# GeekAlexis/FastMOT

Hardware: AMD Instinct MI355X
Metric: end-to-end tracker FPS @1080p/50 dets (higher is better)
Workload: dtype f16

## Files before the change

fastmot_amd/_lib.py:

```python
import ctypes as C
import os
import sys
import weakref
from pathlib import Path

import numpy as np
from types import SimpleNamespace

from .utils.nv12 import NV12Frame
from .utils.jpeg import JPEGFrame, QT_ENTRIES, max_coefficients
from .utils.source import SourceFrame
from .utils.yuv import PlanarFrame, frame_bytes
from .utils.packed import PackedFrame, row_bytes
from .utils.bayer import BayerFrame
from .utils.deep import DeepFrame, deep_frame_bytes
from .utils.devarray import DeviceArrayFrame

LIB_PATH = Path(os.environ.get('FASTMOT_LIB_PATH', Path(__file__).parent / 'libfastmot_hip.so'))

c_int_p = C.POINTER(C.c_int)
_lib = None


class FastMOTHipError(RuntimeError):
# ... 396 lines not shown
        n_trk = len(arrs[1]) + len(arrs[3])
        out = np.empty(CASCADE_HEADER + 3 * n_trk + 3 * len(arrs[6]), np.int32)
        return cin, arrs, out

    def assoc_cascade(self, pack):
        cin, _, out = pack
        check(self.lib.fm_assoc_cascade(self._ctx, C.byref(cin), _ptr(out), C.c_int(len(out))))
        return out[:out[9]].tolist()

    def assoc_get_pairwise(self, nT, nD):
        feat = np.empty((nT, nD), np.float64)
        maha = np.empty((nT, nD), np.float64)
        iou = np.empty((nT, nD), np.float64)
        check(self.lib.fm_assoc_get_pairwise(self._ctx, _ptr(feat), _ptr(maha), _ptr(iou)))
        return feat, maha, iou

    def assoc_stage(self, stage, solver, rows, cols, motion_weight=0., max_cost=0., fill_val=1.,
                    row_labels=None, want_cost=False):
        r = _as(rows, np.int32)
        c = _as(cols, np.int32)
        nr, nc = len(r), len(c)
        mn = min(nr, nc)
        m_rows = np.empty(mn, np.int32)
        m_cols = np.empty(mn, np.int32)
        gated = np.zeros(mn, np.uint8)
        n_match = C.c_int(0)
        cost = np.empty((nr, nc), np.float64) if want_cost else None
        rl = _as(row_labels, np.int64) if row_labels is not None else None
        check(self.lib.fm_assoc_stage(self._ctx, C.c_int(stage), C.c_int(solver), C.c_int(nr), _ptr(r),
                                      C.c_int(nc), _ptr(c), C.c_double(motion_weight),
# ... 798 lines not shown
```

fastmot_amd/csrc/assoc.hip:

```cpp
#include "common.h"
#include "numba_set.h"
#include <algorithm>
#include <cmath>

namespace {

constexpr double INF_COST = 1e5;
constexpr double CHI_SQ_INV_95 = 9.4877;

__device__ inline double box_area(const double* b) {
    const double w = b[2] - b[0] + 1, h = b[3] - b[1] + 1;
    return (w <= 0 || h <= 0) ? 0. : w * h;
}

__device__ inline double iou_dist_pair(const double* a, double area_a, const double* b) {
    const double iw = fmin(a[2], b[2]) - fmax(a[0], b[0]) + 1;
    const double ih = fmin(a[3], b[3]) - fmax(a[1], b[1]) + 1;
    if (iw > 0 && ih > 0) {
        const double inter = iw * ih;
        const double uni = area_a + box_area(b) - inter;
        return 1. - inter / uni;
    }
    return 1.;
}
// ... 23 lines not shown
        }
        __syncthreads();
    }
    if (live) out[i] = occ;
}

__global__ void iou_dist_kernel(int na, const double* __restrict__ a, int nb,
                                const double* __restrict__ b, double* __restrict__ out) {
    const int idx = blockIdx.x * blockDim.x + threadIdx.x;
    if (idx >= na * nb) return;
    const int i = idx / nb, j = idx % nb;
    const double* pa = a + (size_t)i * 4;
    out[idx] = iou_dist_pair(pa, box_area(pa), b + (size_t)j * 4);
}

__global__ __launch_bounds__(256) void pairwise_kernel(
    int nT, int nD, int metric, int dim, const int32_t* __restrict__ slots,
    const double* __restrict__ trk_tlbr, const double* __restrict__ det_tlbr,
    const double* __restrict__ mean, const double* __restrict__ cov,
    const float* __restrict__ favg, const int32_t* __restrict__ fcnt,
    const float* __restrict__ emb, KFConst kf, const uint8_t* __restrict__ row_f32,
    double* __restrict__ feat, double* __restrict__ maha, double* __restrict__ iou,
    uint8_t* __restrict__ row_has_feat, char* __restrict__ mirror) {
    const size_t mat = (size_t)nT * nD;
    double* const mfeat = reinterpret_cast<double*>(mirror);
    extern __shared__ __attribute__((aligned(16))) char smem[];
    float* sa = reinterpret_cast<float*>(smem);
    double* sd = reinterpret_cast<double*>(smem + (size_t)dim * 4);
    const int t = blockIdx.x, tid = threadIdx.x;
    const int slot = slots[t];
    const int cnt = fcnt[slot];
    for (int k = tid; k < dim; k += 256) sa[k] = favg[(size_t)slot * dim + k];
    if (tid == 0) {
        const double* m = mean + (size_t)slot * 8;
        const double* P = cov + (size_t)slot * 64;
        const double w = m[2] - m[0] + 1, h = m[3] - m[1] + 1;
        const double sw = fmax(kf.fac_det[0] * w, kf.min_det[0]);
        const double sh = fmax(kf.fac_det[1] * h, kf.min_det[1]);
        double S[4][4], L[4][4];
        for (int i = 0; i < 4; ++i)
            for (int j = 0; j < 4; ++j) {
                S[i][j] = P[i * 8 + j];
                L[i][j] = 0.;
            }
        S[0][0] += sw * sw; S[1][1] += sh * sh; S[2][2] += sw * sw; S[3][3] += sh * sh;
        for (int j = 0; j < 4; ++j) {
            double s = S[j][j];
            for (int k = 0; k < j; ++k) s -= L[j][k] * L[j][k];
            L[j][j] = sqrt(s);
            for (int i = j + 1; i < 4; ++i) {
                double v = S[i][j];
                for (int k = 0; k < j; ++k) v -= L[i][k] * L[j][k];
                L[i][j] = v / L[j][j];
            }
        }
        for (int i = 0; i < 4; ++i) {
            for (int j = 0; j < 4; ++j) sd[i * 4 + j] = L[i][j];
            sd[16 + i] = m[i];
            sd[20 + i] = trk_tlbr[(size_t)t * 4 + i];
        }
        sd[24] = box_area(trk_tlbr + (size_t)t * 4);
        row_has_feat[t] = cnt > 0 ? 1 : 0;
        if (mirror) reinterpret_cast<uint8_t*>(mfeat + 3 * mat)[t] = cnt > 0 ? 1 : 0;
    }
    __syncthreads();
    for (int d = tid; d < nD; d += 256) {
        const double* z = det_tlbr + (size_t)d * 4;
        double y[4];
        for (int i = 0; i < 4; ++i) {
            double s = z[i] - sd[16 + i];
            for (int k = 0; k < i; ++k) s -= sd[i * 4 + k] * y[k];
            y[i] = s / sd[i * 4 + i];
        }
        const double md = y[0] * y[0] + y[1] * y[1] + y[2] * y[2] + y[3] * y[3];
        const double io = iou_dist_pair(sd + 20, sd[24], z);
        maha[(size_t)t * nD + d] = md;
        iou[(size_t)t * nD + d] = io;
        if (mirror) {
            mfeat[mat + (size_t)t * nD + d] = md;
            mfeat[2 * mat + (size_t)t * nD + d] = io;
        }
    }
    const int wv = tid >> 6, lane = tid & 63;
    const bool f32row = row_f32[t] != 0;
    if (cnt > 0) {
        for (int d = wv; d < nD; d += 4) {
            const float* b = emb + (size_t)d * dim;
            double acc0 = 0., acc1 = 0., acc2 = 0.;
            for (int k4 = lane; k4 < dim / 4; k4 += 64) {
                const float4 bv = *reinterpret_cast<const float4*>(b + k4 * 4);
                const float4 av = *reinterpret_cast<const float4*>(sa + k4 * 4);
                const float af[4] = {av.x, av.y, av.z, av.w};
                const float bf[4] = {bv.x, bv.y, bv.z, bv.w};
#pragma unroll
                for (int e = 0; e < 4; ++e) {
                    if (metric == FM_METRIC_COSINE) {
                        acc2 += (double)(bf[e] * bf[e]);
                        if (f32row) {
                            acc0 += (double)(af[e] * bf[e]);
                            acc1 += (double)(af[e] * af[e]);
                        } else {
                            const double a = af[e];
                            acc0 += a * (double)bf[e];
                            acc1 += a * a;
                        }
                    } else if (f32row) {
                        const float df = af[e] - bf[e];
                        acc0 += (double)(df * df);
                    } else {
                        const double dd = (double)af[e] - (double)bf[e];
                        acc0 += dd * dd;
                    }
                }
            }
            for (int off = 32; off > 0; off >>= 1) {
                acc0 += __shfl_xor(acc0, off);
                acc1 += __shfl_xor(acc1, off);
                acc2 += __shfl_xor(acc2, off);
            }
            if (lane == 0) {
                double v;
                if (metric == FM_METRIC_COSINE) v = 1. - acc0 / (sqrt(acc1) * sqrt(acc2));
                else v = sqrt(acc0);
                feat[(size_t)t * nD + d] = v;
                if (mirror) mfeat[(size_t)t * nD + d] = v;
            }
        }
    } else {
        for (int d = tid; d < nD; d += 256) {
            feat[(size_t)t * nD + d] = 1.;
            if (mirror) mfeat[(size_t)t * nD + d] = 1.;
        }
    }
}

__host__ __device__ inline double stage_cost(int stage, int t, int d, int nD, const double* __restrict__ feat,
                                             const double* __restrict__ maha, const double* __restrict__ iou,
                                             const uint8_t* __restrict__ row_has_feat, const uint8_t* __restrict__ docc,
                                             int64_t rlab, int64_t dlab, double motion_weight, double max_cost,
                                             double fill_val) {
    const size_t p = (size_t)t * nD + d;
    const bool lab_bad = rlab != dlab;
    double c;
    if (stage == FM_STAGE_MATCHING) {
        const bool empty = (!row_has_feat[t]) || docc[d];
        const double f = empty ? fill_val : feat[p];
// ... 500 lines not shown
    std::vector<size_t> offs;
    char* in = nullptr;
    int rc = upload(ctx, ctx->as_in,
                    {{slots, sizeof(int32_t) * nT}, {trk_tlbr, sizeof(double) * 4 * nT},
                     {trk_label, sizeof(int64_t) * nT}, {det_tlbr, sizeof(double) * 4 * nD},
                     {det_label, sizeof(int64_t) * nD}, {det_occluded, (size_t)nD},
                     {trk_feat_f32, (size_t)nT}}, offs, &in, early);
    if (rc) return rc;
    for (int i = 0; i < 6; ++i) ctx->as_off[i] = offs[i];
    const size_t mat = sizeof(double) * (size_t)nT * nD;
    if ((rc = ctx->as_pair.reserve(3 * mat + nT + 64))) return rc;
    char* pr = ctx->as_pair.dev<char>();
    const size_t shmem = (size_t)ctx->feat_dim * 4 + 32 * sizeof(double);
    if (after_extractor && !early) FM_HIP(hipStreamWaitEvent(ctx->s_main, ctx->ev_ext_net, 0));
    fm_trace_mark(ctx, st, 54);
    hipLaunchKernelGGL(pairwise_kernel, dim3(nT), dim3(256), shmem, st, nT, nD, metric,
                       ctx->feat_dim, (const int32_t*)(in + offs[0]), (const double*)(in + offs[1]),
                       (const double*)(in + offs[3]), ctx->mean, ctx->cov, ctx->feat_avg, ctx->feat_cnt,
                       ctx->emb, ctx->kf, (const uint8_t*)(in + offs[6]), (double*)pr, (double*)(pr + mat),
                       (double*)(pr + 2 * mat),
                       (uint8_t*)(pr + 3 * mat), mirror ? ctx->as_pair.host<char>() : nullptr);
    FM_HIP(hipGetLastError());
    fm_trace_mark(ctx, st, 55);
    if (mirror) FM_HIP(hipEventRecord(ctx->ev_pair, st));
    ctx->as_mirror = mirror;
    ctx->as_in_device = !early;
    ctx->as_in_bytes = offs[6] + (size_t)nT;
    return 0;
}

extern "C" int fm_assoc_prepare(fm_ctx* ctx, int metric, int nT, const int32_t* slots,
                                const double* trk_tlbr, const int64_t* trk_label, int nD,
                                const double* det_tlbr, const int64_t* det_label,
                                const uint8_t* det_occluded, const uint8_t* trk_feat_f32) {
    return assoc_prepare_impl(ctx, metric, nT, slots, trk_tlbr, trk_label, nD, det_tlbr, det_label, det_occluded,
                              trk_feat_f32, false);
// ... 250 lines not shown
}

extern "C" int fm_assoc_get_pairwise(fm_ctx* ctx, double* feat, double* maha, double* iou) {
    FM_CHECK_ARG(ctx);
    const size_t mat = sizeof(double) * (size_t)ctx->as_nT * ctx->as_nD;
    if (mat == 0) return 0;
    FM_HIP(hipStreamSynchronize(ctx->s_main));
    if (!ctx->as_in_device) FM_HIP(hipStreamSynchronize(ctx->s_ext));
    char* pr = ctx->as_pair.dev<char>();
    if (feat) FM_HIP(hipMemcpy(feat, pr, mat, hipMemcpyDeviceToHost));
    if (maha) FM_HIP(hipMemcpy(maha, pr + mat, mat, hipMemcpyDeviceToHost));
    if (iou) FM_HIP(hipMemcpy(iou, pr + 2 * mat, mat, hipMemcpyDeviceToHost));
    return 0;
}

extern "C" int fm_assoc_stage(fm_ctx* ctx, int stage, int solver, int nr, const int32_t* rows, int nc,
                              const int32_t* cols, double motion_weight, double max_cost,
                              double fill_val, const int64_t* row_label_override, int32_t* m_rows,
                              int32_t* m_cols, uint8_t* match_gated, int* n_match, double* cost_out) {
    FM_CHECK_ARG(ctx && n_match && nr >= 0 && nc >= 0);
    FM_CHECK_ARG(stage >= FM_STAGE_MATCHING && stage <= FM_STAGE_REID && (solver == 0 || solver == 1));
    *n_match = 0;
    if (nr == 0 || nc == 0) return 0;
    FM_CHECK_ARG(rows && cols && m_rows && m_cols);
    for (int i = 0; i < nr; ++i) FM_CHECK_ARG(rows[i] >= 0 && rows[i] < ctx->as_nT);
    for (int j = 0; j < nc; ++j) FM_CHECK_ARG(cols[j] >= 0 && cols[j] < ctx->as_nD);
    std::vector<int64_t> rlab(nr);
    if (row_label_override) memcpy(rlab.data(), row_label_override, sizeof(int64_t) * nr);
    else {
        const int64_t* tl = reinterpret_cast<const int64_t*>(ctx->as_in.host<char>() + ctx->as_off[2]);
// ... 37 lines not shown
```

fastmot_amd/csrc/common.h:

```cpp
#pragma once
#include <hip/hip_runtime.h>
#include <atomic>
#include <cstdarg>
#include <cstdint>
#include <cstdio>
#include <cstring>
#include <string>
#include <vector>
#include "../../include/fastmot_hip.h"
#ifdef FM_DIAG
#include "../../include/fastmot_hip_diag.h"
#endif

#define FM_ERR_HIP (-1)
#define FM_ERR_ARG (-2)
#define FM_ERR_STATE (-3)

void fm_set_error(const char* fmt, ...);

#define FM_HIP(call)                                                                        \
    do {                                                                                    \
        hipError_t e_ = (call);                                                             \
        if (e_ != hipSuccess) {                                                             \
            fm_set_error("%s:%d %s -> %s", __FILE__, __LINE__, #call, hipGetErrorString(e_)); \
// ... 61 lines not shown
struct SsdState;
struct GalleryState;
constexpr int FM_GALLERY_CHANNELS = 2;

struct fm_ctx {
    int device = 0;
    int opt_zero_copy_tracks = 2048;
    int opt_host_lap_elems = 262144;
    int opt_use_graphs = 1;
    int opt_fused_input = 1;
    int opt_net_timing = 0;
    int opt_nms_general = 0;
    int opt_det_front_ahead = 1;
    int opt_det_front_layers = -1;
    int opt_det_front_stream = 0;
    bool det_flush_deferred = false;
    int opt_lk_variant = 0;
    void* predict_worker = nullptr;
    hipStream_t s_main = nullptr;
    hipStream_t s_det = nullptr;
    hipStream_t s_up = nullptr;
    hipStream_t s_ext = nullptr;
    hipStream_t s_ext_x[FM_MAX_EXTRA_EXTRACTORS] = {};
    hipEvent_t ev_ext_in = nullptr, ev_ext_x_done[FM_MAX_EXTRA_EXTRACTORS] = {};
    hipStream_t s_flow = nullptr;
    hipStream_t s_flow2 = nullptr;
    hipEvent_t ev_pyr = nullptr;
    bool pyr_pending = false;
    hipEvent_t ev_prep = nullptr, ev_bg = nullptr;
    hipEvent_t ev_feat = nullptr;
// ... 186 lines not shown
```

fastmot_amd/csrc/ctx.hip:

```cpp
#include <algorithm>
#include "common.h"
void convd_set_cfg(int code);
#include <sched.h>
#include <cstring>
#include <cstdlib>
#include <cmath>

static thread_local char g_err[1024] = "";

void fm_set_error(const char* fmt, ...) {
    va_list ap;
    va_start(ap, fmt);
    vsnprintf(g_err, sizeof(g_err), fmt, ap);
    va_end(ap);
}

extern "C" const char* fm_last_error(void) { return g_err; }

extern "C" int fm_ctx_set_option(fm_ctx* ctx, const char* key, int value) {
    FM_CHECK_ARG(ctx && key && (value >= 0 || (value == -1 && !strcmp(key, "det_front_layers"))));
    if (!strcmp(key, "zero_copy_tracks")) ctx->opt_zero_copy_tracks = value;
    else if (!strcmp(key, "host_lap_elems")) ctx->opt_host_lap_elems = value;
    else if (!strcmp(key, "use_graphs")) ctx->opt_use_graphs = value;
    else if (!strcmp(key, "convd_cfg")) convd_set_cfg(value);
    else if (!strcmp(key, "nms_path")) {
        ctx->opt_nms_general = value != 0;
    }
    else if (!strcmp(key, "fused_input")) ctx->opt_fused_input = value != 0;
    else if (!strcmp(key, "net_timing")) ctx->opt_net_timing = value;
    else if (!strcmp(key, "det_front_ahead") || !strcmp(key, "det_front_stream")) {
        FM_CHECK_ARG(value <= (key[10] == 'a' ? 2 : 1));
        (key[10] == 'a' ? ctx->opt_det_front_ahead : ctx->opt_det_front_stream) = value;
    }
    else if (!strcmp(key, "det_front_layers")) ctx->opt_det_front_layers = value;
    else if (!strcmp(key, "lk_variant")) {
#ifndef FM_DIAG
        if (value != 0) {
            fm_set_error("option 'lk_variant' needs a diagnostic build of the library (-DFM_DIAG)");
            return FM_ERR_ARG;
        }
#endif
        ctx->opt_lk_variant = value;
    }
    else {
        fm_set_error("unknown option '%s'", key);
        return FM_ERR_ARG;
    }
    return 0;
}

extern "C" int fm_ctx_get_option(fm_ctx* ctx, const char* key, int* value) {
    FM_CHECK_ARG(ctx && key && value);
    if (!strcmp(key, "det_front_ahead")) *value = ctx->opt_det_front_ahead;
    else if (!strcmp(key, "det_front_layers")) *value = ctx->opt_det_front_layers;
    else if (!strcmp(key, "det_front_stream")) *value = ctx->opt_det_front_stream;
    else {
        fm_set_error("option '%s' cannot be read", key);
        return FM_ERR_ARG;
    }
    return 0;
}

extern "C" int fm_trace_start(fm_ctx* ctx, int cap, int64_t* host_ns) {
    FM_CHECK_ARG(ctx && cap > 0 && host_ns && !ctx->trace_on.load() && ctx->trace_ev.empty());
    FM_HIP(hipDeviceSynchronize());
    std::vector<hipEvent_t> evs(cap);
    for (auto& e : evs) FM_HIP(hipEventCreate(&e));
    if (!ctx->trace_base) FM_HIP(hipEventCreate(&ctx->trace_base));
    FM_HIP(hipEventRecord(ctx->trace_base, ctx->s_main));
    FM_HIP(hipEventSynchronize(ctx->trace_base));
// ... 54 lines not shown
    int n = 0;
    FM_HIP(hipGetDeviceCount(&n));
    if (device < 0 || device >= n) {
        fm_set_error("device %d out of range (%d visible)", device, n);
        return FM_ERR_ARG;
    }
    FM_HIP(hipSetDevice(device));
    fm_ctx* ctx = new fm_ctx();
    ctx->device = device;
    if (const char* e = getenv("FASTMOT_ZERO_COPY")) ctx->opt_zero_copy_tracks = atoi(e);
    if (const char* e = getenv("FASTMOT_HOST_LAP")) ctx->opt_host_lap_elems = atoi(e);
    if (const char* e = getenv("FASTMOT_GRAPHS")) ctx->opt_use_graphs = atoi(e);
    if (const char* e = getenv("FASTMOT_FUSED_INPUT")) ctx->opt_fused_input = atoi(e) != 0;
    if (const char* e = getenv("FASTMOT_FRONT_AHEAD")) ctx->opt_det_front_ahead = std::min(std::max(atoi(e), 0), 2);
    if (const char* e = getenv("FASTMOT_FRONT_STREAM")) ctx->opt_det_front_stream = atoi(e) == 1;
    int prio_lo = 0, prio_hi = 0;
    FM_HIP(hipDeviceGetStreamPriorityRange(&prio_lo, &prio_hi));
    const int prio_det = prio_lo, prio_ext = prio_hi;
    FM_HIP(hipStreamCreateWithPriority(&ctx->s_main, hipStreamNonBlocking, prio_hi));
    FM_HIP(hipStreamCreateWithPriority(&ctx->s_det, hipStreamNonBlocking, prio_det));
    FM_HIP(hipStreamCreateWithPriority(&ctx->s_up, hipStreamNonBlocking, prio_lo));
    FM_HIP(hipStreamCreateWithPriority(&ctx->s_ext, hipStreamNonBlocking, prio_ext));
    FM_HIP(hipEventCreateWithFlags(&ctx->ev_ext_in, hipEventDisableTiming));
    for (int i = 0; i < FM_MAX_EXTRA_EXTRACTORS; ++i) {
        FM_HIP(hipStreamCreateWithPriority(&ctx->s_ext_x[i], hipStreamNonBlocking, prio_hi));
        FM_HIP(hipEventCreateWithFlags(&ctx->ev_ext_x_done[i], hipEventDisableTiming));
    }
    FM_HIP(hipStreamCreateWithPriority(&ctx->s_flow, hipStreamNonBlocking, prio_hi));
    FM_HIP(hipStreamCreateWithPriority(&ctx->s_flow2, hipStreamNonBlocking, prio_hi));
    FM_HIP(hipEventCreateWithFlags(&ctx->ev_pyr, hipEventDisableTiming));
// ... 411 lines not shown
```

fastmot_amd/csrc/detect.hip:

```cpp
#include "pixel_source.h"
#include <cmath>
#include <string>
#include <vector>

struct DetState {
    fm_yolo_cfg cfg{};
    bool configured = false;
    int cap = 8192;
    static constexpr int NSLOT_UNTILED = FM_MAX_DET_BATCH + 2;
    static constexpr int NSLOT = 3 * FM_MAX_DET_BATCH;
    int nslot = NSLOT_UNTILED;
    int n_tiles = 0;
    int tile_x[FM_MAX_DET_BATCH] = {}, tile_y[FM_MAX_DET_BATCH] = {};
    int region_w = 0, region_h = 0;
    double tile_offset[FM_MAX_DET_BATCH][2] = {};
    double merge_thresh = 0.6;
    std::vector<fm_det48> tile_stage;
    std::vector<fm_det48> tile_dets;
    std::vector<int32_t> tile_ids;
    int tile_count[FM_MAX_DET_BATCH] = {};
    int tile_sum[2] = {};
    float* cand[NSLOT] = {};
    float* sorted[NSLOT] = {};
    int32_t* counters[NSLOT] = {};
    uint64_t* mask[NSLOT] = {};
    fm_det48* dets[NSLOT] = {};
    bool used[NSLOT] = {};
    hipEvent_t ev_dec[NSLOT] = {};
    int post_pending = -1;
    int post_pending_n = 0;
    bool general_post = false;
    static constexpr int GREEDY_RETRY = 1024;
    int general_passes = 0;
    int greedy_kmax = 2048, greedy_shrink = 0;
    bool sorted_valid[NSLOT] = {};
    static constexpr int PREFIX = 2048;
    fm_det48* dets_host[NSLOT] = {};
    int32_t* counters_host[NSLOT] = {};
    hipEvent_t ev_done[NSLOT] = {};
    hipStream_t s_fallback = nullptr;
    hipEvent_t ev0[NSLOT] = {}, ev1[NSLOT] = {};
    bool timed[NSLOT] = {};
    hipEvent_t evf0[NSLOT] = {}, evf1[NSLOT] = {};
    bool timed_front[NSLOT] = {};
    hipEvent_t ev_front[2] = {};
// ... 151 lines not shown
    const int i = blockIdx.x * blockDim.x + threadIdx.x;
    if (i >= n) return;
    const float* r = rows + (size_t)i * 7;
    emit_candidate(fa, r[0], r[1], r[2], r[3], r[4], (int)r[5], r[6], i);
}

#include "nms_core.h"

}
bool fm_det_defers_flush(fm_ctx* ctx) {
    return ctx->det && ctx->det_net && ctx->det_net->front_k > 0 && ctx->opt_det_front_ahead && ctx->opt_det_front_layers &&
           ctx->opt_det_front_stream == 0;
}
namespace {

int ensure_det(fm_ctx* ctx) {
    if (ctx->det) return 0;
    ctx->det = new DetState();
    return 0;
}

int alloc_post(DetState* d, int cap, int nslot) {
    cap = (cap + 63) & ~63;
    if (d->cand[0] && cap == d->cap && nslot == d->nslot) return 0;
    for (int i = (cap != d->cap || !d->cand[0]) ? 0 : nslot; i < DetState::NSLOT; ++i) {
        for (void* p : {(void*)d->cand[i], (void*)d->sorted[i], (void*)d->mask[i], (void*)d->dets[i]})
            if (p) (void)hipFree(p);
        if (d->dets_host[i]) (void)hipHostFree(d->dets_host[i]);
        d->dets_host[i] = nullptr;
        d->cand[i] = d->sorted[i] = nullptr; d->mask[i] = nullptr; d->dets[i] = nullptr;
    }
    for (int i = 0; i < DetState::NSLOT; ++i) d->used[i] = false;
    d->cap = cap;
    d->nslot = nslot;
    d->wr = d->rd = d->pending = 0;
    d->last = -1;
    d->post_pending = -1;
    d->post_pending_n = 0;
    d->set_slot[0] = d->set_slot[1] = -1;
    for (int i = 0; i < nslot; ++i) {
        if (d->cand[i]) continue;
        FM_HIP(hipMalloc(&d->cand[i], sizeof(float) * 8 * cap));
        FM_HIP(hipMalloc(&d->sorted[i], sizeof(float) * 8 * cap));
        FM_HIP(hipMalloc(&d->mask[i], sizeof(uint64_t) * (size_t)cap * (cap / 64)));
        FM_HIP(hipMalloc(&d->dets[i], sizeof(fm_det48) * cap));
        FM_HIP(hipHostMalloc(&d->dets_host[i], sizeof(fm_det48) * cap, hipHostMallocDefault));
    }
    for (int i = 0; i < nslot; ++i) {
        if (d->counters[i]) continue;
        FM_HIP(hipMalloc(&d->counters[i], sizeof(int32_t) * 4));
        FM_HIP(hipHostMalloc(&d->counters_host[i], sizeof(int32_t) * 4, hipHostMallocDefault));
        FM_HIP(hipEventCreateWithFlags(&d->ev_done[i], hipEventDisableTiming));
        FM_HIP(hipEventCreateWithFlags(&d->ev_dec[i], hipEventDisableTiming));
// ... 67 lines not shown
}

static int enqueue_greedy_post(fm_ctx* ctx, DetState* d, int slot, hipStream_t sp) {
    static bool configured = false;
    if (int rc = allow_dynamic_lds(nms_greedy_kernel, ng_lds_bytes(NG_KMAX), configured)) return rc;
    int rc = launch_rank_sort(d, slot, sp);
    if (rc) return rc;
    fm_trace_mark(ctx, sp, 22);
    const int kmax = d->greedy_kmax < d->cap ? d->greedy_kmax : (d->cap < NG_KMAX ? d->cap : NG_KMAX);
    hipLaunchKernelGGL(nms_greedy_kernel, dim3(1), dim3(NG_T), ng_lds_bytes(kmax), sp, d->sorted[slot], d->counters[slot],
                       d->cap, kmax, d->cfg.nms_thresh, post_out(d, slot));
    FM_HIP(hipGetLastError());
    return 0;
}

static int flush_post(fm_ctx* ctx, DetState* d) {
    const int first = d->post_pending, n = d->post_pending_n;
    if (first < 0) return 0;
    d->post_pending = -1;
    d->post_pending_n = 0;
    hipStream_t sp = ctx->s_up;
    FM_HIP(hipStreamWaitEvent(sp, d->ev_dec[first], 0));
    for (int i = 0; i < n; ++i) {
        const int slot = (first + i) % d->nslot;
        fm_trace_mark(ctx, sp, 20);
        int rc_p = (d->general_post || ctx->opt_nms_general) ? enqueue_general_post(ctx, d, slot, sp) : enqueue_greedy_post(ctx, d, slot, sp);
        if (rc_p) return rc_p;
        FM_HIP(hipEventRecord(d->ev_done[slot], sp));
        fm_trace_mark(ctx, sp, 21);
    }
    return 0;
}

int enqueue_post(fm_ctx* ctx, DetState* d, hipStream_t s, int n = 1) {
    int rc = flush_post(ctx, d);
    if (rc) return rc;
    while (d->pending + n > d->nslot) {
        const int drop = d->n_tiles > 1 ? d->n_tiles : 1;
        d->rd = (d->rd + drop) % d->nslot;
        d->pending -= drop;
    }
    const int slot = d->wr;
    FM_HIP(hipEventRecord(d->ev_dec[slot], s));
    d->post_pending = slot;
    d->post_pending_n = n;
    for (int i = 0; i < n; ++i) d->used[(slot + i) % d->nslot] = true;
    d->wr = (slot + n) % d->nslot;
    d->pending += n;
    return 0;
}

static int acquire_slots(fm_ctx* ctx, DetState* d, hipStream_t s, int n = 1) {
    if (d->post_pending >= 0 && d->post_pending_n + n > d->nslot) {
        int rc = flush_post(ctx, d);
        if (rc) return rc;
    }
    for (int i = 0; i < n; ++i) {
        const int slot = (d->wr + i) % d->nslot;
        if (d->used[slot] && hipEventQuery(d->ev_done[slot]) != hipSuccess) {
            (void)hipGetLastError();
            FM_HIP(hipStreamWaitEvent(s, d->ev_done[slot], 0));
        }
    }
    return 0;
}

int collect(fm_ctx* ctx, DetState* d, hipStream_t s, fm_det48* out, int cap_out, int* n) {
    if (d->pending == 0) {
        fm_set_error("no detector pass in flight (fm_detect_async first)");
        return FM_ERR_STATE;
    }
    const int slot = d->rd;
    bool later = d->post_pending >= 0 && (slot - d->post_pending + d->nslot) % d->nslot >= d->post_pending_n && fm_det_defers_flush(ctx);
    if (later && hipEventQuery(d->ev_dec[d->post_pending]) == hipSuccess) later = false;
    (void)hipGetLastError();
    if (!later) {
        int rc_f = flush_post(ctx, d);
        if (rc_f) return rc_f;
    }
    FM_HIP(hipEventSynchronize(d->ev_done[slot]));
    if (d->counters_host[slot][3] != 0 && !d->counters_host[slot][1]) {
        const int why = d->counters_host[slot][3];
        if (!d->s_fallback) FM_HIP(hipStreamCreateWithFlags(&d->s_fallback, hipStreamNonBlocking));
        hipStream_t sp = d->s_fallback;
        int rc_g = enqueue_general_post(ctx, d, slot, sp, d->sorted_valid[slot]);
        if (rc_g) return rc_g;
        FM_HIP(hipStreamSynchronize(sp));
// ... 97 lines not shown
extern "C" int fm_detect_configure(fm_ctx* ctx, const fm_yolo_cfg* cfg) {
    FM_CHECK_ARG(ctx && cfg);
    FM_CHECK_ARG(cfg->n_heads >= 0 && cfg->n_heads <= FM_MAX_HEADS && cfg->num_classes > 0 && cfg->num_classes <= 128);
    {
        long long rows = 0;
        for (int i = 0; i < cfg->n_heads; ++i) {
            FM_CHECK_ARG(cfg->n_anchors[i] > 0 && cfg->n_anchors[i] <= FM_MAX_ANCHORS && cfg->grid_w[i] > 0 && cfg->grid_h[i] > 0);
            rows += (long long)cfg->grid_w[i] * cfg->grid_h[i] * cfg->n_anchors[i];
        }
        FM_CHECK_ARG(rows < (1ll << FM_SORT_INDEX_BITS));
    }
    int rc = ensure_det(ctx);
    if (rc) return rc;
    DetState* d = ctx->det;
    FM_HIP(hipStreamSynchronize(ctx->s_det));
    FM_HIP(hipStreamSynchronize(ctx->s_up));
    if (int rc_n = fm_net_sync(ctx->det_net)) return rc_n;
    d->set_slot[0] = d->set_slot[1] = -1;
    d->post_pending = -1;
    d->post_pending_n = 0;
    d->rd = d->wr;
    d->pending = 0;
    d->cfg = *cfg;
    d->general_post = ctx->opt_nms_general != 0;
    d->n_tiles = 0;
    d->tile_dets.clear();
    d->tile_ids.clear();
    if ((rc = alloc_post(d, cfg->max_candidates > 0 ? cfg->max_candidates : 8192, DetState::NSLOT_UNTILED))) return rc;
    FM_HIP(hipMemcpy(d->label_mask, cfg->label_mask, 128, hipMemcpyHostToDevice));
    d->configured = true;
    return 0;
}

extern "C" int fm_detect_configure_tiles(fm_ctx* ctx, int n_tiles, const int32_t* origins, int region_w, int region_h,
                                         const double* offsets, double merge_thresh) {
    FM_CHECK_ARG(ctx && ctx->det && ctx->det->configured);
    FM_CHECK_ARG(n_tiles == 0 || (n_tiles >= 2 && n_tiles <= FM_MAX_DET_BATCH));
    DetState* d = ctx->det;
    if (n_tiles) {
        FM_CHECK_ARG(origins && offsets && region_w > 0 && region_h > 0 && merge_thresh >= 0. && merge_thresh <= 1.);
        for (int t = 0; t < n_tiles; ++t)
            FM_CHECK_ARG(origins[2 * t] >= 0 && origins[2 * t + 1] >= 0 && origins[2 * t] + d->cfg.in_w <= region_w &&
                         origins[2 * t + 1] + d->cfg.in_h <= region_h);
    }
    FM_HIP(hipStreamSynchronize(ctx->s_det));
    FM_HIP(hipStreamSynchronize(ctx->s_up));
    if (int rc_n = fm_net_sync(ctx->det_net)) return rc_n;
    d->set_slot[0] = d->set_slot[1] = -1;
    d->post_pending = -1;
    d->post_pending_n = 0;
    d->rd = d->wr;
    d->pending = 0;
    d->tile_dets.clear();
    d->tile_ids.clear();
    d->n_tiles = n_tiles;
    for (int t = 0; t < n_tiles; ++t) {
        d->tile_x[t] = origins[2 * t]; d->tile_y[t] = origins[2 * t + 1];
        d->tile_offset[t][0] = offsets[2 * t]; d->tile_offset[t][1] = offsets[2 * t + 1];
        d->tile_count[t] = 0;
    }
    if (n_tiles) {
        d->region_w = region_w; d->region_h = region_h;
        d->merge_thresh = merge_thresh;
    }
    d->last = -1;
// ... 145 lines not shown
        fm_net_select(net, se, set);
        if (timing) FM_HIP(hipEventRecord(d->evf0[d->wr], se));
        fm_trace_mark(ctx, se, 11);
        if ((rc = fm_net_run_stem_from(ctx, net, src, n))) return rc;
        fm_trace_mark(ctx, se, 15);
        if (K > 1) {
            net->first = 1;
            net->last = K;
            if ((rc = fm_net_run_internal(ctx, FM_NET_DETECTOR, n))) return rc;
        }
        if (timing) FM_HIP(hipEventRecord(d->evf1[d->wr], se));
        fm_trace_mark(ctx, se, 16);
        FM_HIP(hipEventRecord(d->ev_front[set], se));
        if (ctx->det_flush_deferred) {
            ctx->det_flush_deferred = false;
            if ((rc = flush_post(ctx, d))) return rc;
        }
        fm_net_select(net, nullptr, set);
        FM_HIP(hipStreamWaitEvent(s, d->ev_front[set], 0));
        fm_trace_mark(ctx, s, 14);
        if (timing) FM_HIP(hipEventRecord(d->ev0[d->wr], s));
        net->first = K;
        net->last = 0;
        if ((rc = fm_net_run_internal(ctx, FM_NET_DETECTOR, n))) return rc;
        net->first = 0;
    } else {
        for (int i = 0; i < n_frames; ++i)
            if (uploads[i]) FM_HIP(hipStreamWaitEvent(s, uploads[i], 0));
        if ((rc = acquire_slots(ctx, d, s, n))) return rc;
        fm_trace_mark(ctx, s, 14);
        const StemSrc src = det_source(ctx, d, frames, n);
// ... 50 lines not shown
    return enqueue_post(ctx, d, s, n);
}

extern "C" int fm_detect_sync(fm_ctx* ctx, fm_det48* out, int cap, int* n) {
    FM_CHECK_ARG(ctx && ctx->det && ctx->det->configured && out && n);
    if (ctx->det->n_tiles > 1) return collect_tiles(ctx, ctx->det, ctx->s_det, out, cap, n);
    return collect(ctx, ctx->det, ctx->s_det, out, cap, n);
}

extern "C" int fm_filter_dets(fm_ctx* ctx, const float* rows, int n, fm_det48* out, int cap, int* n_out) {
    FM_CHECK_ARG(ctx && ctx->det && ctx->det->configured && n >= 0 && out && n_out);
    FM_CHECK_ARG(n < (1 << FM_SORT_INDEX_BITS));
    DetState* d = ctx->det;
    hipStream_t s = ctx->s_det;
    FM_HIP(hipStreamSynchronize(s));
    FM_HIP(hipStreamSynchronize(ctx->s_up));
    if (int rc_n = fm_net_sync(ctx->det_net)) return rc_n;
    d->set_slot[0] = d->set_slot[1] = -1;
    d->post_pending = -1;
    d->post_pending_n = 0;
    d->rd = d->wr;
    d->pending = 0;
    if (n > d->rows_cap) {
        if (d->rows_in) FM_HIP(hipFree(d->rows_in));
        d->rows_in = nullptr;
        FM_HIP(hipMalloc(&d->rows_in, sizeof(float) * 7 * (size_t)n));
        d->rows_cap = n;
    }
    if (n) FM_HIP(hipMemcpyAsync(d->rows_in, rows, sizeof(float) * 7 * (size_t)n, hipMemcpyHostToDevice, s));
    FM_HIP(hipMemsetAsync(d->counters[d->wr], 0, sizeof(int32_t) * 4, s));
    if (n) hipLaunchKernelGGL(rows_filter_kernel, dim3((n + 255) / 256), dim3(256), 0, s, d->rows_in, n, filter_args(d, d->wr));
    int rc = enqueue_post(ctx, d, s);
    if (rc) return rc;
    return collect(ctx, d, s, out, cap, n_out);
}
// ... 19 lines not shown
    FM_CHECK_ARG(ctx && ctx->det && out && counts && n_tiles);
    const DetState* d = ctx->det;
    FM_CHECK_ARG(d->n_tiles > 1 && (int)d->tile_dets.size() <= cap);
    if (!d->tile_dets.empty()) memcpy(out, d->tile_dets.data(), sizeof(fm_det48) * d->tile_dets.size());
    for (int t = 0; t < d->n_tiles; ++t) counts[t] = d->tile_count[t];
    *n_tiles = d->n_tiles;
    return 0;
}

extern "C" int fm_detect_raw_candidates(fm_ctx* ctx, float* rows, int cap, int* n) {
    FM_CHECK_ARG(ctx && ctx->det && rows && n);
    DetState* d = ctx->det;
    int rc_f = flush_post(ctx, d);
    if (rc_f) return rc_f;
    FM_HIP(hipStreamSynchronize(ctx->s_det));
    FM_HIP(hipStreamSynchronize(ctx->s_up));
    if (int rc_n = fm_net_sync(ctx->det_net)) return rc_n;
    const int slot = (d->wr + d->nslot - 1) % d->nslot;
    int32_t cnt[4];
    FM_HIP(hipMemcpy(cnt, d->counters[slot], sizeof(cnt), hipMemcpyDeviceToHost));
    const int k = cnt[0] < d->cap ? cnt[0] : d->cap;
    FM_CHECK_ARG(k <= cap);
    FM_HIP(hipMemcpy(rows, d->sorted[slot], sizeof(float) * 8 * k, hipMemcpyDeviceToHost));
    *n = k;
    return 0;
}

extern "C" int fm_detect_net_ms(fm_ctx* ctx, float* ms) {
    FM_CHECK_ARG(ctx && ctx->det && ms && ctx->det->last >= 0);
    const int slot = ctx->det->last;
    if (!ctx->det->timed[slot]) { *ms = -1.f; return 0; }
// ... 10 lines not shown
```

include/fastmot_hip.h:

```cpp
#ifndef FASTMOT_HIP_H
#define FASTMOT_HIP_H

#include <stddef.h>
#include <stdint.h>

#ifdef __cplusplus
extern "C" {
#endif

typedef struct fm_ctx fm_ctx;

int fm_ctx_create(int device, fm_ctx** out);
int fm_ctx_destroy(fm_ctx* ctx);
const char* fm_last_error(void);
int fm_device_count(void);
int fm_device_pci_bus_id(int device, char* buf, int buflen);
int fm_ctx_synchronize(fm_ctx* ctx);
int fm_ctx_bind_thread(fm_ctx* ctx);
int fm_ctx_set_option(fm_ctx* ctx, const char* key, int value);
int fm_ctx_get_option(fm_ctx* ctx, const char* key, int* value);
int fm_net_front_info(fm_ctx* ctx, int* k, long long* bytes, long long* passes);
int fm_trace_start(fm_ctx* ctx, int cap, int64_t* host_ns);
int fm_trace_read(fm_ctx* ctx, int cap, int32_t* tags, float* ms, int* n);
int fm_device_info(fm_ctx* ctx, char* buf, int buflen);
// ... 35 lines not shown
int fm_feat_reset(fm_ctx* ctx, int n, const int32_t* slots);
int fm_feat_get(fm_ctx* ctx, int slot, float* sum, float* avg, int32_t* count);
int fm_feat_read(fm_ctx* ctx, int n, const int32_t* slots, float* avg_out, int32_t* count_out);
int fm_feat_write(fm_ctx* ctx, int n, const int32_t* slots, const float* avg, const int32_t* count);

enum { FM_METRIC_EUCLIDEAN = 0, FM_METRIC_COSINE = 1 };

int fm_find_occluded(fm_ctx* ctx, int n, const double* tlbr, double thresh, uint8_t* out);

int fm_assoc_prepare(fm_ctx* ctx, int metric,
                     int nT, const int32_t* slots, const double* trk_tlbr, const int64_t* trk_label,
                     int nD, const double* det_tlbr, const int64_t* det_label,
                     const uint8_t* det_occluded, const uint8_t* trk_feat_f32);

int fm_assoc_get_pairwise(fm_ctx* ctx, double* feat, double* maha, double* iou);

enum {
    FM_STAGE_MATCHING = 0,
    FM_STAGE_IOU      = 1,
    FM_STAGE_REID     = 2
};

int fm_assoc_stage(fm_ctx* ctx, int stage, int solver,
                   int nr, const int32_t* rows, int nc, const int32_t* cols,
                   double motion_weight, double max_cost, double fill_val,
                   const int64_t* row_label_override,
                   int32_t* m_rows, int32_t* m_cols, uint8_t* match_gated, int* n_match,
                   double* cost_out);

int fm_assoc_prepare2(fm_ctx* ctx, int metric,
// ... 492 lines not shown
```

Measured before the change: 1073.

## Split pairwise kernel across detection parts and add optional post-process stream modes

Changes the pairwise association kernel to use a 2D grid, with one y-block computing Mahalanobis/IoU and optional extra y-blocks splitting the feature-distance loop over detections. The inner loop now loads two float4s per iteration. Also adds options to run detector post-processing on the extractor stream or defer it, plus new host APIs for reading row_has_feat and the pinned mirror. Both new options default to 0, so the default path is one block per track with the restructured kernel. That block now handles Mahalanobis, IoU and features in sequence, with an extra barrier.

```diff
diff --git a/fastmot_amd/_lib.py b/fastmot_amd/_lib.py
--- a/fastmot_amd/_lib.py
+++ b/fastmot_amd/_lib.py
@@ -434,6 +434,19 @@
         iou = np.empty((nT, nD), np.float64)
         check(self.lib.fm_assoc_get_pairwise(self._ctx, _ptr(feat), _ptr(maha), _ptr(iou)))
         return feat, maha, iou
+
+    def assoc_get_row_has_feat(self, nT):
+        has = np.zeros(nT, np.uint8)
+        check(self.lib.fm_assoc_get_row_has_feat(self._ctx, _ptr(has)))
+        return has
+
+    def assoc_get_pairwise_mirror(self, nT, nD):
+        feat = np.empty((nT, nD), np.float64)
+        maha = np.empty((nT, nD), np.float64)
+        iou = np.empty((nT, nD), np.float64)
+        has = np.zeros(nT, np.uint8)
+        check(self.lib.fm_assoc_get_pairwise_mirror(self._ctx, _ptr(feat), _ptr(maha), _ptr(iou), _ptr(has)))
+        return feat, maha, iou, has
 
     def assoc_stage(self, stage, solver, rows, cols, motion_weight=0., max_cost=0., fill_val=1.,
                     row_labels=None, want_cost=False):
diff --git a/fastmot_amd/csrc/assoc.hip b/fastmot_amd/csrc/assoc.hip
--- a/fastmot_amd/csrc/assoc.hip
+++ b/fastmot_amd/csrc/assoc.hip
@@ -61,6 +61,7 @@
     out[idx] = iou_dist_pair(pa, box_area(pa), b + (size_t)j * 4);
 }
 
+
 __global__ __launch_bounds__(256) void pairwise_kernel(
     int nT, int nD, int metric, int dim, const int32_t* __restrict__ slots,
     const double* __restrict__ trk_tlbr, const double* __restrict__ det_tlbr,
@@ -68,77 +69,96 @@
     const float* __restrict__ favg, const int32_t* __restrict__ fcnt,
     const float* __restrict__ emb, KFConst kf, const uint8_t* __restrict__ row_f32,
     double* __restrict__ feat, double* __restrict__ maha, double* __restrict__ iou,
-    uint8_t* __restrict__ row_has_feat, char* __restrict__ mirror) {
+    uint8_t* __restrict__ row_has_feat, char* __restrict__ mirror, int np) {
     const size_t mat = (size_t)nT * nD;
     double* const mfeat = reinterpret_cast<double*>(mirror);
     extern __shared__ __attribute__((aligned(16))) char smem[];
     float* sa = reinterpret_cast<float*>(smem);
     double* sd = reinterpret_cast<double*>(smem + (size_t)dim * 4);
     const int t = blockIdx.x, tid = threadIdx.x;
+    const int part = np ? blockIdx.y : 0, parts = np ? np : 1;
     const int slot = slots[t];
     const int cnt = fcnt[slot];
+    if ((int)blockIdx.y == np) {
+        if (tid == 0) {
+            const double* m = mean + (size_t)slot * 8;
+            const double* P = cov + (size_t)slot * 64;
+            const double w = m[2] - m[0] + 1, h = m[3] - m[1] + 1;
+            const double sw = fmax(kf.fac_det[0] * w, kf.min_det[0]);
+            const double sh = fmax(kf.fac_det[1] * h, kf.min_det[1]);
+            double S[4][4], L[4][4];
+            for (int i = 0; i < 4; ++i)
+                for (int j = 0; j < 4; ++j) {
+                    S[i][j] = P[i * 8 + j];
+                    L[i][j] = 0.;
+                }
+            S[0][0] += sw * sw; S[1][1] += sh * sh; S[2][2] += sw * sw; S[3][3] += sh * sh;
+            for (int j = 0; j < 4; ++j) {
+                double s = S[j][j];
+                for (int k = 0; k < j; ++k) s -= L[j][k] * L[j][k];
+                L[j][j] = sqrt(s);
+                for (int i = j + 1; i < 4; ++i) {
+                    double v = S[i][j];
+                    for (int k = 0; k < j; ++k) v -= L[i][k] * L[j][k];
+                    L[i][j] = v / L[j][j];
+                }
+            }
+            for (int i = 0; i < 4; ++i) {
+                for (int j = 0; j < 4; ++j) sd[i * 4 + j] = L[i][j];
+                sd[16 + i] = m[i];
+                sd[20 + i] = trk_tlbr[(size_t)t * 4 + i];
+            }
+            sd[24] = box_area(trk_tlbr + (size_t)t * 4);
+            row_has_feat[t] = cnt > 0 ? 1 : 0;
+            if (mirror) reinterpret_cast<uint8_t*>(mfeat + 3 * mat)[t] = cnt > 0 ? 1 : 0;
+        }
+        __syncthreads();
+        for (int d = tid; d < nD; d += 256) {
+            const double* z = det_tlbr + (size_t)d * 4;
+            double y[4];
+            for (int i = 0; i < 4; ++i) {
+                double s = z[i] - sd[16 + i];
+                for (int k = 0; k < i; ++k) s -= sd[i * 4 + k] * y[k];
+                y[i] = s / sd[i * 4 + i];
+            }
+            const double md = y[0] * y[0] + y[1] * y[1] + y[2] * y[2] + y[3] * y[3];
+            const double io = iou_dist_pair(sd + 20, sd[24], z);
+            maha[(size_t)t * nD + d] = md;
+            iou[(size_t)t * nD + d] = io;
+            if (mirror) {
+                mfeat[mat + (size_t)t * nD + d] = md;
+                mfeat[2 * mat + (size_t)t * nD + d] = io;
+            }
+        }
+        if (np) return;
+    }
+    if (4 * part >= nD) return;
+    if (cnt <= 0) {
+        for (int d = tid + 256 * part; d < nD; d += 256 * parts) {
+            feat[(size_t)t * nD + d] = 1.;
+            if (mirror) mfeat[(size_t)t * nD + d] = 1.;
+        }
+        return;
+    }
     for (int k = tid; k < dim; k += 256) sa[k] = favg[(size_t)slot * dim + k];
-    if (tid == 0) {
-        const double* m = mean + (size_t)slot * 8;
-        const double* P = cov + (size_t)slot * 64;
-        const double w = m[2] - m[0] + 1, h = m[3] - m[1] + 1;
-        const double sw = fmax(kf.fac_det[0] * w, kf.min_det[0]);
-        const double sh = fmax(kf.fac_det[1] * h, kf.min_det[1]);
-        double S[4][4], L[4][4];
-        for (int i = 0; i < 4; ++i)
-            for (int j = 0; j < 4; ++j) {
-                S[i][j] = P[i * 8 + j];
-                L[i][j] = 0.;
-            }
-        S[0][0] += sw * sw; S[1][1] += sh * sh; S[2][2] += sw * sw; S[3][3] += sh * sh;
-        for (int j = 0; j < 4; ++j) {
-            double s = S[j][j];
-            for (int k = 0; k < j; ++k) s -= L[j][k] * L[j][k];
-            L[j][j] = sqrt(s);
-            for (int i = j + 1; i < 4; ++i) {
-                double v = S[i][j];
-                for (int k = 0; k < j; ++k) v -= L[i][k] * L[j][k];
-                L[i][j] = v / L[j][j];
-            }
-        }
-        for (int i = 0; i < 4; ++i) {
-            for (int j = 0; j < 4; ++j) sd[i * 4 + j] = L[i][j];
-            sd[16 + i] = m[i];
-            sd[20 + i] = trk_tlbr[(size_t)t * 4 + i];
-        }
-        sd[24] = box_area(trk_tlbr + (size_t)t * 4);
-        row_has_feat[t] = cnt > 0 ? 1 : 0;
-        if (mirror) reinterpret_cast<uint8_t*>(mfeat + 3 * mat)[t] = cnt > 0 ? 1 : 0;
-    }
-    __syncthreads();
-    for (int d = tid; d < nD; d += 256) {
-        const double* z = det_tlbr + (size_t)d * 4;
-        double y[4];
-        for (int i = 0; i < 4; ++i) {
-            double s = z[i] - sd[16 + i];
-            for (int k = 0; k < i; ++k) s -= sd[i * 4 + k] * y[k];
-            y[i] = s / sd[i * 4 + i];
-        }
-        const double md = y[0] * y[0] + y[1] * y[1] + y[2] * y[2] + y[3] * y[3];
-        const double io = iou_dist_pair(sd + 20, sd[24], z);
-        maha[(size_t)t * nD + d] = md;
-        iou[(size_t)t * nD + d] = io;
-        if (mirror) {
-            mfeat[mat + (size_t)t * nD + d] = md;
-            mfeat[2 * mat + (size_t)t * nD + d] = io;
-        }
-    }
     const int wv = tid >> 6, lane = tid & 63;
     const bool f32row = row_f32[t] != 0;
-    if (cnt > 0) {
-        for (int d = wv; d < nD; d += 4) {
-            const float* b = emb + (size_t)d * dim;
-            double acc0 = 0., acc1 = 0., acc2 = 0.;
-            for (int k4 = lane; k4 < dim / 4; k4 += 64) {
-                const float4 bv = *reinterpret_cast<const float4*>(b + k4 * 4);
-                const float4 av = *reinterpret_cast<const float4*>(sa + k4 * 4);
+    const int n4 = dim / 4;
+    __syncthreads();
+    for (int d = wv + 4 * part; d < nD; d += 4 * parts) {
+        const float* b = emb + (size_t)d * dim;
+        double acc0 = 0., acc1 = 0., acc2 = 0.;
+        for (int k4 = lane; k4 < n4; k4 += 128) {
+            const int n = k4 + 64 < n4 ? 2 : 1;
+            float4 bv[2];
+            bv[0] = *reinterpret_cast<const float4*>(b + k4 * 4);
+            bv[1] = n == 2 ? *reinterpret_cast<const float4*>(b + (k4 + 64) * 4) : make_float4(0.f, 0.f, 0.f, 0.f);
+#pragma unroll
+            for (int h = 0; h < 2; ++h) {
+                if (h >= n) break;
+                const float4 av = *reinterpret_cast<const float4*>(sa + (k4 + 64 * h) * 4);
                 const float af[4] = {av.x, av.y, av.z, av.w};
-                const float bf[4] = {bv.x, bv.y, bv.z, bv.w};
+                const float bf[4] = {bv[h].x, bv[h].y, bv[h].z, bv[h].w};
 #pragma unroll
                 for (int e = 0; e < 4; ++e) {
                     if (metric == FM_METRIC_COSINE) {
@@ -160,23 +180,18 @@
                     }
                 }
             }
-            for (int off = 32; off > 0; off >>= 1) {
-                acc0 += __shfl_xor(acc0, off);
-                acc1 += __shfl_xor(acc1, off);
-                acc2 += __shfl_xor(acc2, off);
-            }
-            if (lane == 0) {
-                double v;
-                if (metric == FM_METRIC_COSINE) v = 1. - acc0 / (sqrt(acc1) * sqrt(acc2));
-                else v = sqrt(acc0);
-                feat[(size_t)t * nD + d] = v;
-                if (mirror) mfeat[(size_t)t * nD + d] = v;
-            }
-        }
-    } else {
-        for (int d = tid; d < nD; d += 256) {
-            feat[(size_t)t * nD + d] = 1.;
-            if (mirror) mfeat[(size_t)t * nD + d] = 1.;
+        }
+        for (int off = 32; off > 0; off >>= 1) {
+            acc0 += __shfl_xor(acc0, off);
+            acc1 += __shfl_xor(acc1, off);
+            acc2 += __shfl_xor(acc2, off);
+        }
+        if (lane == 0) {
+            double v;
+            if (metric == FM_METRIC_COSINE) v = 1. - acc0 / (sqrt(acc1) * sqrt(acc2));
+            else v = sqrt(acc0);
+            feat[(size_t)t * nD + d] = v;
+            if (mirror) mfeat[(size_t)t * nD + d] = v;
         }
     }
 }
@@ -707,12 +722,12 @@
     const size_t shmem = (size_t)ctx->feat_dim * 4 + 32 * sizeof(double);
     if (after_extractor && !early) FM_HIP(hipStreamWaitEvent(ctx->s_main, ctx->ev_ext_net, 0));
     fm_trace_mark(ctx, st, 54);
-    hipLaunchKernelGGL(pairwise_kernel, dim3(nT), dim3(256), shmem, st, nT, nD, metric,
+    hipLaunchKernelGGL(pairwise_kernel, dim3(nT, 1 + ctx->opt_pairwise_parts), dim3(256), shmem, st, nT, nD, metric,
                        ctx->feat_dim, (const int32_t*)(in + offs[0]), (const double*)(in + offs[1]),
                        (const double*)(in + offs[3]), ctx->mean, ctx->cov, ctx->feat_avg, ctx->feat_cnt,
                        ctx->emb, ctx->kf, (const uint8_t*)(in + offs[6]), (double*)pr, (double*)(pr + mat),
                        (double*)(pr + 2 * mat),
-                       (uint8_t*)(pr + 3 * mat), mirror ? ctx->as_pair.host<char>() : nullptr);
+                       (uint8_t*)(pr + 3 * mat), mirror ? ctx->as_pair.host<char>() : nullptr, ctx->opt_pairwise_parts);
     FM_HIP(hipGetLastError());
     fm_trace_mark(ctx, st, 55);
     if (mirror) FM_HIP(hipEventRecord(ctx->ev_pair, st));
@@ -993,6 +1008,33 @@
     return 0;
 }
 
+extern "C" int fm_assoc_get_row_has_feat(fm_ctx* ctx, uint8_t* row_has_feat) {
+    FM_CHECK_ARG(ctx && row_has_feat);
+    const size_t mat = sizeof(double) * (size_t)ctx->as_nT * ctx->as_nD;
+    if (mat == 0) return 0;
+    FM_HIP(hipStreamSynchronize(ctx->s_main));
+    if (!ctx->as_in_device) FM_HIP(hipStreamSynchronize(ctx->s_ext));
+    FM_HIP(hipMemcpy(row_has_feat, ctx->as_pair.dev<char>() + 3 * mat, (size_t)ctx->as_nT, hipMemcpyDeviceToHost));
+    return 0;
+}
+
+extern "C" int fm_assoc_get_pairwise_mirror(fm_ctx* ctx, double* feat, double* maha, double* iou, uint8_t* row_has_feat) {
+    FM_CHECK_ARG(ctx);
+    const size_t mat = sizeof(double) * (size_t)ctx->as_nT * ctx->as_nD;
+    if (mat == 0) return 0;
+    if (!ctx->as_mirror) {
+        fm_set_error("the pairwise terms of this frame have no page-locked mirror");
+        return FM_ERR_STATE;
+    }
+    FM_HIP(hipEventSynchronize(ctx->ev_pair));
+    const char* pm = ctx->as_pair.host<char>();
+    if (feat) memcpy(feat, pm, mat);
+    if (maha) memcpy(maha, pm + mat, mat);
+    if (iou) memcpy(iou, pm + 2 * mat, mat);
+    if (row_has_feat) memcpy(row_has_feat, pm + 3 * mat, (size_t)ctx->as_nT);
+    return 0;
+}
+
 extern "C" int fm_assoc_stage(fm_ctx* ctx, int stage, int solver, int nr, const int32_t* rows, int nc,
                               const int32_t* cols, double motion_weight, double max_cost,
                               double fill_val, const int64_t* row_label_override, int32_t* m_rows,
diff --git a/fastmot_amd/csrc/common.h b/fastmot_amd/csrc/common.h
--- a/fastmot_amd/csrc/common.h
+++ b/fastmot_amd/csrc/common.h
@@ -99,6 +99,8 @@
     int opt_det_front_ahead = 1;
     int opt_det_front_layers = -1;
     int opt_det_front_stream = 0;
+    int opt_pairwise_parts = 0;
+    int opt_det_post_stream = 0;
     bool det_flush_deferred = false;
     int opt_lk_variant = 0;
     void* predict_worker = nullptr;
diff --git a/fastmot_amd/csrc/ctx.hip b/fastmot_amd/csrc/ctx.hip
--- a/fastmot_amd/csrc/ctx.hip
+++ b/fastmot_amd/csrc/ctx.hip
@@ -33,6 +33,14 @@
         (key[10] == 'a' ? ctx->opt_det_front_ahead : ctx->opt_det_front_stream) = value;
     }
     else if (!strcmp(key, "det_front_layers")) ctx->opt_det_front_layers = value;
+    else if (!strcmp(key, "pairwise_parts")) {
+        FM_CHECK_ARG(value <= 16);
+        ctx->opt_pairwise_parts = value;
+    }
+    else if (!strcmp(key, "det_post_stream")) {
+        FM_CHECK_ARG(value <= 2);
+        ctx->opt_det_post_stream = value;
+    }
     else if (!strcmp(key, "lk_variant")) {
 #ifndef FM_DIAG
         if (value != 0) {
@@ -54,6 +62,8 @@
     if (!strcmp(key, "det_front_ahead")) *value = ctx->opt_det_front_ahead;
     else if (!strcmp(key, "det_front_layers")) *value = ctx->opt_det_front_layers;
     else if (!strcmp(key, "det_front_stream")) *value = ctx->opt_det_front_stream;
+    else if (!strcmp(key, "det_post_stream")) *value = ctx->opt_det_post_stream;
+    else if (!strcmp(key, "pairwise_parts")) *value = ctx->opt_pairwise_parts;
     else {
         fm_set_error("option '%s' cannot be read", key);
         return FM_ERR_ARG;
@@ -138,6 +148,8 @@
     if (const char* e = getenv("FASTMOT_FUSED_INPUT")) ctx->opt_fused_input = atoi(e) != 0;
     if (const char* e = getenv("FASTMOT_FRONT_AHEAD")) ctx->opt_det_front_ahead = std::min(std::max(atoi(e), 0), 2);
     if (const char* e = getenv("FASTMOT_FRONT_STREAM")) ctx->opt_det_front_stream = atoi(e) == 1;
+    if (const char* e = getenv("FASTMOT_PAIRWISE_PARTS")) ctx->opt_pairwise_parts = std::min(std::max(atoi(e), 0), 16);
+    if (const char* e = getenv("FASTMOT_POST_STREAM")) ctx->opt_det_post_stream = std::min(std::max(atoi(e), 0), 2);
     int prio_lo = 0, prio_hi = 0;
     FM_HIP(hipDeviceGetStreamPriorityRange(&prio_lo, &prio_hi));
     const int prio_det = prio_lo, prio_ext = prio_hi;
diff --git a/fastmot_amd/csrc/detect.hip b/fastmot_amd/csrc/detect.hip
--- a/fastmot_amd/csrc/detect.hip
+++ b/fastmot_amd/csrc/detect.hip
@@ -29,6 +29,8 @@
     hipEvent_t ev_dec[NSLOT] = {};
     int post_pending = -1;
     int post_pending_n = 0;
+    int post_late = -1, post_late_n = 0;
+    bool post_on_ext = false;
     bool general_post = false;
     static constexpr int GREEDY_RETRY = 1024;
     int general_passes = 0;
@@ -210,6 +212,12 @@
 }
 namespace {
 
+int sync_post(fm_ctx* ctx, DetState* d) {
+    FM_HIP(hipStreamSynchronize(ctx->s_up));
+    if (d->post_on_ext) FM_HIP(hipStreamSynchronize(ctx->s_ext));
+    return 0;
+}
+
 int ensure_det(fm_ctx* ctx) {
     if (ctx->det) return 0;
     ctx->det = new DetState();
@@ -231,8 +239,8 @@
     d->nslot = nslot;
     d->wr = d->rd = d->pending = 0;
     d->last = -1;
-    d->post_pending = -1;
-    d->post_pending_n = 0;
+    d->post_pending = d->post_late = -1;
+    d->post_pending_n = d->post_late_n = 0;
     d->set_slot[0] = d->set_slot[1] = -1;
     for (int i = 0; i < nslot; ++i) {
         if (d->cand[i]) continue;
@@ -330,13 +338,24 @@
     return 0;
 }
 
-static int flush_post(fm_ctx* ctx, DetState* d) {
+static int flush_post(fm_ctx* ctx, DetState* d, hipStream_t sp = nullptr, bool decoded = false, bool keep_late = false) {
+    if (d->post_late >= 0 && !decoded && !keep_late) {
+        const int p = d->post_pending, pn = d->post_pending_n;
+        d->post_pending = d->post_late;
+        d->post_pending_n = d->post_late_n;
+        d->post_late = -1;
+        int rc_l = flush_post(ctx, d);
+        d->post_pending = p;
+        d->post_pending_n = pn;
+        if (rc_l) return rc_l;
+    }
     const int first = d->post_pending, n = d->post_pending_n;
     if (first < 0) return 0;
     d->post_pending = -1;
     d->post_pending_n = 0;
-    hipStream_t sp = ctx->s_up;
-    FM_HIP(hipStreamWaitEvent(sp, d->ev_dec[first], 0));
+    if (!sp) sp = ctx->s_up;
+    if (sp == ctx->s_ext) d->post_on_ext = true;
+    if (!decoded) FM_HIP(hipStreamWaitEvent(sp, d->ev_dec[first], 0));
     for (int i = 0; i < n; ++i) {
         const int slot = (first + i) % d->nslot;
         fm_trace_mark(ctx, sp, 20);
@@ -349,7 +368,7 @@
 }
 
 int enqueue_post(fm_ctx* ctx, DetState* d, hipStream_t s, int n = 1) {
-    int rc = flush_post(ctx, d);
+    int rc = flush_post(ctx, d, nullptr, false, true);
     if (rc) return rc;
     while (d->pending + n > d->nslot) {
         const int drop = d->n_tiles > 1 ? d->n_tiles : 1;
@@ -367,7 +386,7 @@
 }
 
 static int acquire_slots(fm_ctx* ctx, DetState* d, hipStream_t s, int n = 1) {
-    if (d->post_pending >= 0 && d->post_pending_n + n > d->nslot) {
+    if (d->post_late >= 0 || (d->post_pending >= 0 && d->post_pending_n + n > d->nslot)) {
         int rc = flush_post(ctx, d);
         if (rc) return rc;
     }
@@ -387,6 +406,17 @@
         return FM_ERR_STATE;
     }
     const int slot = d->rd;
+    if (d->post_late >= 0 && (slot - d->post_late + d->nslot) % d->nslot < d->post_late_n) {
+        const int p = d->post_pending, pn = d->post_pending_n;
+        FM_HIP(hipEventSynchronize(d->ev_dec[d->post_late]));
+        d->post_pending = d->post_late;
+        d->post_pending_n = d->post_late_n;
+        d->post_late = -1;
+        int rc_l = flush_post(ctx, d, ctx->s_ext, true);
+        d->post_pending = p;
+        d->post_pending_n = pn;
+        if (rc_l) return rc_l;
+    }
     bool later = d->post_pending >= 0 && (slot - d->post_pending + d->nslot) % d->nslot >= d->post_pending_n && fm_det_defers_flush(ctx);
     if (later && hipEventQuery(d->ev_dec[d->post_pending]) == hipSuccess) later = false;
     (void)hipGetLastError();
@@ -514,11 +544,11 @@
     if (rc) return rc;
     DetState* d = ctx->det;
     FM_HIP(hipStreamSynchronize(ctx->s_det));
-    FM_HIP(hipStreamSynchronize(ctx->s_up));
+    if (int rc_s = sync_post(ctx, d)) return rc_s;
     if (int rc_n = fm_net_sync(ctx->det_net)) return rc_n;
     d->set_slot[0] = d->set_slot[1] = -1;
-    d->post_pending = -1;
-    d->post_pending_n = 0;
+    d->post_pending = d->post_late = -1;
+    d->post_pending_n = d->post_late_n = 0;
     d->rd = d->wr;
     d->pending = 0;
     d->cfg = *cfg;
@@ -544,11 +574,11 @@
                          origins[2 * t + 1] + d->cfg.in_h <= region_h);
     }
     FM_HIP(hipStreamSynchronize(ctx->s_det));
-    FM_HIP(hipStreamSynchronize(ctx->s_up));
+    if (int rc_s = sync_post(ctx, d)) return rc_s;
     if (int rc_n = fm_net_sync(ctx->det_net)) return rc_n;
     d->set_slot[0] = d->set_slot[1] = -1;
-    d->post_pending = -1;
-    d->post_pending_n = 0;
+    d->post_pending = d->post_late = -1;
+    d->post_pending_n = d->post_late_n = 0;
     d->rd = d->wr;
     d->pending = 0;
     d->tile_dets.clear();
@@ -724,7 +754,12 @@
         FM_HIP(hipEventRecord(d->ev_front[set], se));
         if (ctx->det_flush_deferred) {
             ctx->det_flush_deferred = false;
-            if ((rc = flush_post(ctx, d))) return rc;
+            if (ctx->opt_det_post_stream == 2 && se == ctx->s_up && d->post_pending >= 0 && d->post_late < 0) {
+                d->post_late = d->post_pending;
+                d->post_late_n = d->post_pending_n;
+                d->post_pending = -1;
+                d->post_pending_n = 0;
+            } else if ((rc = flush_post(ctx, d, ctx->opt_det_post_stream == 1 && se == ctx->s_up ? ctx->s_ext : nullptr))) return rc;
         }
         fm_net_select(net, nullptr, set);
         FM_HIP(hipStreamWaitEvent(s, d->ev_front[set], 0));
@@ -805,11 +840,11 @@
     DetState* d = ctx->det;
     hipStream_t s = ctx->s_det;
     FM_HIP(hipStreamSynchronize(s));
-    FM_HIP(hipStreamSynchronize(ctx->s_up));
+    if (int rc_s = sync_post(ctx, d)) return rc_s;
     if (int rc_n = fm_net_sync(ctx->det_net)) return rc_n;
     d->set_slot[0] = d->set_slot[1] = -1;
-    d->post_pending = -1;
-    d->post_pending_n = 0;
+    d->post_pending = d->post_late = -1;
+    d->post_pending_n = d->post_late_n = 0;
     d->rd = d->wr;
     d->pending = 0;
     if (n > d->rows_cap) {
@@ -859,7 +894,7 @@
     int rc_f = flush_post(ctx, d);
     if (rc_f) return rc_f;
     FM_HIP(hipStreamSynchronize(ctx->s_det));
-    FM_HIP(hipStreamSynchronize(ctx->s_up));
+    if (int rc_s = sync_post(ctx, d)) return rc_s;
     if (int rc_n = fm_net_sync(ctx->det_net)) return rc_n;
     const int slot = (d->wr + d->nslot - 1) % d->nslot;
     int32_t cnt[4];
diff --git a/include/fastmot_hip.h b/include/fastmot_hip.h
--- a/include/fastmot_hip.h
+++ b/include/fastmot_hip.h
@@ -73,6 +73,8 @@
                      const uint8_t* det_occluded, const uint8_t* trk_feat_f32);
 
 int fm_assoc_get_pairwise(fm_ctx* ctx, double* feat, double* maha, double* iou);
+int fm_assoc_get_row_has_feat(fm_ctx* ctx, uint8_t* row_has_feat);
+int fm_assoc_get_pairwise_mirror(fm_ctx* ctx, double* feat, double* maha, double* iou, uint8_t* row_has_feat);
 
 enum {
     FM_STAGE_MATCHING = 0,
```

Result: no change. 1071, median of 3 (-0.1%).
